# vmskisme/f_renderer

Hardware: AMD Instinct MI355X
Metric: Mtri/s (and Mfrag/s), 1M-triangle frame @1920x1080 (higher is better)
Workload: dtype f32; 1 GPU; random_1M_tris_1920x1080_depth; scene=1M random clip-space triangles, 1920x1080, depth-only, width=1920, height=1080, triangles=1000000, setup_triangles=1000052, covered_fragments=60715175, varyings=0, tile=32x32, frames_in_flight=2, partition=tile rows in 1 contiguous block(s)

## Files before the change

f_renderer_amd/csrc/frr_raster.h:

```cpp
#pragma once
#include "frr_device.h"
#ifndef __HIPCC_RTC__
#include <type_traits>
#endif

namespace frr {

__device__ __forceinline__ int xcd_remap(int bid, int nwg)
{
    const int q = nwg / 8, r = nwg % 8, xcd = bid % 8;
    return (xcd < r ? xcd * (q + 1) : r * (q + 1) + (xcd - r) * q) + bid / 8;
}

__device__ __forceinline__ uint32_t order_id(const RasterArgs &a, uint32_t slot)
{
    const uint32_t nt = a.ntris_draw;
    return 1u + (slot < nt ? slot << FAN_BITS : a.fan_okey[slot - nt]);
}
__device__ __forceinline__ uint32_t id_slot(const RasterArgs &a, uint32_t id)
{
    const uint32_t okl = id - 1u, t = okl >> FAN_BITS, f = okl & ((1u << FAN_BITS) - 1u);
    return f ? a.ntris_draw + a.fanbase[t] + (f - 1u) : t;
}
__device__ __forceinline__ uint32_t id_emission(const RasterArgs &a, uint32_t tri_base, uint32_t id)
// ... 209 lines not shown
    const uint32_t A12 = 0u - (uint32_t)(p2y - p1y), B12 = (uint32_t)(p2x - p1x);
    const uint32_t A20 = 0u - (uint32_t)(p0y - p2y), B20 = (uint32_t)(p0x - p2x);
    const uint32_t E01o = A01 * (uint32_t)(bx0 - p0x) + B01 * (uint32_t)(by0 - p0y);
    const uint32_t E12o = A12 * (uint32_t)(bx0 - p1x) + B12 * (uint32_t)(by0 - p1y);
    const uint32_t E20o = A20 * (uint32_t)(bx0 - p2x) + B20 * (uint32_t)(by0 - p2y);
    const uint32_t fl = r->flags;
    const int thr01 = (fl & 2u) ? 0 : -1, thr12 = (fl & 4u) ? 0 : -1, thr20 = (fl & 8u) ? 0 : -1;
    const float r0 = r->rhw[0], r1 = r->rhw[1], r2 = r->rhw[2];
    const float inv_bw = __builtin_amdgcn_rcpf((float)bw);
    const unsigned long long idlow = (unsigned long long)key_id;
    for (int p = lane; p < npx; p += 64) {
        const int dy = (int)(((float)p + 0.5f) * inv_bw);
        const int dx = p - __mul24(dy, bw);
        const int E01 = (int)(E01o + A01 * (uint32_t)dx + B01 * (uint32_t)dy);
        const int E12 = (int)(E12o + A12 * (uint32_t)dx + B12 * (uint32_t)dy);
        const int E20 = (int)(E20o + A20 * (uint32_t)dx + B20 * (uint32_t)dy);
        bool covered = (E01 > thr01) & (E12 > thr12) & (E20 > thr20);
        const int cx = bx0 + dx, cy = by0 + dy;
        const int pix = (cy - c.ay0) * TILE + (cx - c.ax0);
        if (NANPASS) {
            const uint32_t last_nan = nanL[pix];
            covered = covered && last_nan != 0u && key_id > last_nan;
        } else {
            n_cov += (uint32_t)__popcll(__ballot(covered));
        }
        if (covered) {
            Frag f = frag_eval(s0x, s0y, s1x, s1y, s2x, s2y, r0, r1, r2, cx, cy);
            if (f.valid) {
                const bool isnan = f.rhw != f.rhw;
                if (NANPASS) {
                    if (!isnan) atomicMax(&s_key[pix], ((unsigned long long)zkey(f.rhw) << 32) | idlow);
                } else {
                    if (isnan) { ++n_nan; *nanflag = 1u; }
                    atomicMax(&s_key[pix], ((unsigned long long)zkey_frag(f.rhw) << 32) | idlow);
                }
            }
        }
    }
}

__device__ __forceinline__ void tile_nan_begin(const TileCtx &c, unsigned long long *s_key, uint32_t *nanL)
{
    for (int i = threadIdx.x; i < TILE_PX; i += (int)blockDim.x) {
        const int x = i & (TILE - 1), y = i >> 5;
        const unsigned long long k = s_key[i];
        const bool nanpix = x < c.tw && y < c.th && (uint32_t)(k >> 32) == ZKEY_NAN_FRAG;
        nanL[i] = nanpix ? (uint32_t)k : 0u;
        if (nanpix) s_key[i] = ((unsigned long long)ZKEY_NAN_BELOW << 32) | (unsigned long long)(uint32_t)k;
    }
}

template <int K, int PS>
__global__ __launch_bounds__(256) void k_raster(RasterArgs a, DevUniforms u)
{
    __shared__ unsigned long long s_key[TILE_PX];
    __shared__ uint32_t s_nanL[TILE_PX];
    __shared__ uint32_t s_nanflag;
    if (seq_cancelled(a.cnt, a.seq, a.epoch, true)) return;
    const TileCtx c = tile_ctx(a);
    if (c.beg >= c.end) return;
    tile_load_keys(a, c, s_key);
    if (threadIdx.x == 0) s_nanflag = 0u;
    __syncthreads();
    const int lane = threadIdx.x & 63;
    const uint32_t wave = __builtin_amdgcn_readfirstlane(threadIdx.x >> 6);
    uint32_t n_cov = 0, n_nan = 0;
    for (uint32_t e = c.beg + wave; e < c.end; e += 4) {
        const uint32_t t = __builtin_amdgcn_readfirstlane(a.bins[e].x);
        sweep_triangle(a, c, t, order_id(a, t), lane, s_key, n_cov, n_nan, &s_nanflag);
    }
    if (lane == 0 && n_cov) atomicAdd(&a.cnt->lane[a.lane].gtab[a.gpar].frag_covered, (unsigned long long)n_cov);
    if (n_nan) atomicAdd(&a.cnt->lane[a.lane].gtab[a.gpar].frag_nan, (unsigned long long)n_nan);
    __syncthreads();
    if (s_nanflag != 0u) {
        tile_nan_begin(c, s_key, s_nanL);
        __syncthreads();
        for (uint32_t e = c.beg + wave; e < c.end; e += 4) {
            const uint32_t t = __builtin_amdgcn_readfirstlane(a.bins[e].x);
            sweep_triangle<true>(a, c, t, order_id(a, t), lane, s_key, n_cov, n_nan, nullptr, s_nanL);
        }
        __syncthreads();
    }
    tile_resolve<K, PS>(a, u, c, s_key);
}

template <int K, int PS>
__global__ __launch_bounds__(256) void k_raster_entries(RasterArgs a, DevUniforms u)
{
    if (seq_cancelled(a.cnt, a.seq, a.epoch, true)) return;
    const GeomTab *g = gtab_of(a);
    const uint32_t n = g->n_emit, tri_base = g->tri_base;
    const long long nent = (long long)(a.win_h - 1) * a.dstride + a.win_w;
    const long long e = (long long)blockIdx.x * 256 + threadIdx.x;
    if (e >= nent) return;
    const int ex = (int)(e % a.dstride), ey = (int)(e / a.dstride);
    const int kmax = (a.win_w - 1 - ex) / a.dstride;
    float depth = a.depth[e];
    uint32_t id = 0u, n_cov = 0u, n_nan = 0u;
    bool wrote = false;
    for (uint32_t i = 0; i < n; ++i) {
        const uint32_t t = slot_of_emission(a, i);
        const RasterRec *__restrict__ r = a.recs + t;
        const float s0x = r->s[0], s0y = r->s[1], s1x = r->s[2], s1y = r->s[3], s2x = r->s[4], s2y = r->s[5];
        const int p0x = f32_as_i32(s0x + 0.5f), p0y = f32_as_i32(s0y + 0.5f), p1x = f32_as_i32(s1x + 0.5f), p1y = f32_as_i32(s1y + 0.5f);
        const int p2x = f32_as_i32(s2x + 0.5f), p2y = f32_as_i32(s2y + 0.5f);
        const int bx0 = clampi(min(p0x, min(p1x, p2x)), a.x0, a.x1), bx1 = clampi(max(p0x, max(p1x, p2x)), a.x0, a.x1);
        const int by0 = clampi(min(p0y, min(p1y, p2y)), a.y0, a.y1), by1 = clampi(max(p0y, max(p1y, p2y)), a.y0, a.y1);
        if (bx1 <= bx0 || by1 <= by0) continue;
        const uint32_t A01 = 0u - (uint32_t)(p1y - p0y), B01 = (uint32_t)(p1x - p0x);
        const uint32_t A12 = 0u - (uint32_t)(p2y - p1y), B12 = (uint32_t)(p2x - p1x);
        const uint32_t A20 = 0u - (uint32_t)(p0y - p2y), B20 = (uint32_t)(p0x - p2x);
        const uint32_t fl = r->flags;
        const int thr01 = (fl & 2u) ? 0 : -1, thr12 = (fl & 4u) ? 0 : -1, thr20 = (fl & 8u) ? 0 : -1;
        const float r0 = r->rhw[0], r1 = r->rhw[1], r2 = r->rhw[2];
        for (int k = kmax; k >= 0; --k) {
            const int lx = ex + k * a.dstride, ly = ey - k;
            if (ly < 0 || ly >= a.win_h) continue;
            const int cx = a.x0 + lx, cy = a.y0 + ly;
            if (cx < bx0 || cx >= bx1 || cy < by0 || cy >= by1) continue;
            const int E01 = (int)(A01 * (uint32_t)(cx - p0x) + B01 * (uint32_t)(cy - p0y));
            const int E12 = (int)(A12 * (uint32_t)(cx - p1x) + B12 * (uint32_t)(cy - p1y));
            const int E20 = (int)(A20 * (uint32_t)(cx - p2x) + B20 * (uint32_t)(cy - p2y));
            if (!((E01 > thr01) & (E12 > thr12) & (E20 > thr20))) continue;
            ++n_cov;
            const Frag f = frag_eval(s0x, s0y, s1x, s1y, s2x, s2y, r0, r1, r2, cx, cy);
            if (!f.valid) continue;
            if (f.rhw != f.rhw) ++n_nan;
            if (f.rhw < depth) continue;
            depth = f.rhw; id = tri_base + i; wrote = true;
            if constexpr (PS != FRR_PS_DEPTH) {
                const float w = recip_exact(f.rhw != 0.0f ? f.rhw : 1.0f);
                const float c0 = r0 * f.a * w, c1 = r1 * f.b * w, c2 = r2 * f.c * w;
                float in[K > 0 ? K : 1];
                if constexpr (K > 0) {
                    const float *v = a.vary + (size_t)t * (3 * K);
#pragma unroll
                    for (int q = 0; q < K; ++q) in[q] = v[q] * c0 + v[K + q] * c1 + v[2 * K + q] * c2;
                }
                float col[4];
                run_ps<PS>(u, in, col, nullptr);
                reinterpret_cast<uint32_t *>(a.color)[(size_t)ly * a.cstride + lx] =
                    quantize_u8(col[0]) | (quantize_u8(col[1]) << 8) | (quantize_u8(col[2]) << 16) | (quantize_u8(col[3]) << 24);
            }
        }
    }
    if (wrote) { a.depth[e] = depth; a.tri_id[e] = id; }
    if (n_cov) atomicAdd(&a.cnt->lane[a.lane].gtab[a.gpar].frag_covered, (unsigned long long)n_cov);
    if (n_nan) atomicAdd(&a.cnt->lane[a.lane].gtab[a.gpar].frag_nan, (unsigned long long)n_nan);
}

constexpr int SPAN_SAFE = 8191;
constexpr int SPAN_BATCH = 32;
#ifndef FRR_SPAN_CULL
#define FRR_SPAN_CULL 32
#endif
constexpr int SPAN_CULL = FRR_SPAN_CULL;
#ifndef FRR_SPAN_AQ_MIN
#define FRR_SPAN_AQ_MIN 1
#endif
#ifndef FRR_LIGHT_NW
#define FRR_LIGHT_NW 3
#endif
#ifndef FRR_LIGHT_B
#define FRR_LIGHT_B 32
#endif
constexpr int LIGHT_NW = FRR_LIGHT_NW;
constexpr int LIGHT_B = FRR_LIGHT_B;
constexpr int SPAN_AQ_MIN = FRR_SPAN_AQ_MIN;

__device__ __forceinline__ void wave_lds_fence()
{
    __builtin_amdgcn_fence(__ATOMIC_ACQ_REL, "wavefront");
}

__device__ __forceinline__ int seg_rank(uint32_t h_lo, uint32_t h_hi, uint32_t le_lo, uint32_t le_hi, int base)
{
    return __popc(h_hi & le_hi) + (__popc(h_lo & le_lo) + base);
}
struct alignas(16) SpanTri {
    int32_t m01, m12, m20;
    uint32_t zub;
    uint32_t kd01, kd12, kd20;
    uint32_t misc;
    float r01, r12, r20, pad;
};
__device__ __forceinline__ void span_edge_bound(int m, uint32_t kd, float rD, int pmask, int row, int &lo, int &hi)
{
    const int k = (int)(kd << 16) >> 16, D = (int)(kd >> 16);
    const int M = m + __mul24(k, row);
    int q = (int)__builtin_amdgcn_fmed3f((float)M * rD, -2.0f, 40.0f);
    const int r = M - __mul24(q, D);
    q += (r >> 31) + (int)(r >= D);
    lo = max(lo, q & pmask);
    hi = min(hi, max(q + 1, pmask & 64));
}

constexpr int DIRECT_MAX = 256;
#ifndef FRR_DIRECT_STEPS
#define FRR_DIRECT_STEPS 2
#endif
constexpr int DIRECT_STEPS = FRR_DIRECT_STEPS;
constexpr int DIRECT_MIN = 4;
constexpr int HZ_SEG = 0, HZ_BLK = 128, HZ_QUAD = 144, HZ_C4 = 148, HZ_SIZE = 404;
#ifndef FRR_BKT_LOG2
#define FRR_BKT_LOG2 6
#endif
constexpr int BKT_LOG2 = FRR_BKT_LOG2, BKT_N = 1 << BKT_LOG2, BKT_SHIFT = 27 - BKT_LOG2, BKT_PER = BKT_N / 64;
__device__ __forceinline__ uint32_t z_bucket(uint32_t zub_key) { return (uint32_t)(BKT_N - 1) - ((zub_key >> BKT_SHIFT) & (uint32_t)(BKT_N - 1)); }
__device__ __forceinline__ void bucket_scan(uint32_t *s_bkt, int lane, uint32_t base)
{
    uint32_t v[BKT_PER], sum = 0u;
#pragma unroll
    for (int j = 0; j < BKT_PER; ++j) { v[j] = s_bkt[lane * BKT_PER + j]; sum += v[j]; }
    uint32_t run = base + wave_incl_scan_dpp(sum) - sum;
#pragma unroll
    for (int j = 0; j < BKT_PER; ++j) { s_bkt[lane * BKT_PER + j] = run; run += v[j]; }
}
__device__ __forceinline__ uint32_t dpp_xor1(uint32_t v) { return (uint32_t)__builtin_amdgcn_update_dpp(0, (int)v, 0xB1, 0xf, 0xf, false); }
__device__ __forceinline__ uint32_t dpp_xor2(uint32_t v) { return (uint32_t)__builtin_amdgcn_update_dpp(0, (int)v, 0x4E, 0xf, 0xf, false); }

__device__ __forceinline__ void hiz_rebuild(const unsigned long long *s_key, uint32_t *hz, int lane)
{
    const uint4 *p = reinterpret_cast<const uint4 *>(s_key);
    uint32_t m[8];
#pragma unroll
    for (int k = 0; k < 8; ++k) { const uint4 v = p[64 * k + lane]; m[k] = min(v.y, v.w); }
    uint32_t c4[8], sg[8];
#pragma unroll
    for (int k = 0; k < 8; ++k) {
        c4[k] = min(m[k], dpp_xor1(m[k]));
        sg[k] = min(c4[k], dpp_xor2(c4[k]));
    }
#pragma unroll
    for (int k = 0; k < 8; ++k) {
        if ((lane & 1) == 0) hz[HZ_C4 + 32 * k + (lane >> 1)] = c4[k] >> 1;
        if ((lane & 3) == 0) hz[HZ_SEG + 16 * k + (lane >> 2)] = sg[k];
    }
    __builtin_amdgcn_fence(__ATOMIC_ACQ_REL, "wavefront");
    if (lane < 16) {
        const int by = lane >> 2, bx = lane & 3;
        uint32_t mm = 0xFFFFFFFFu;
#pragma unroll
        for (int r = 0; r < 8; ++r) mm = min(mm, hz[HZ_SEG + (by * 8 + r) * 4 + bx]);
        hz[HZ_BLK + lane] = mm;
    }
    __builtin_amdgcn_fence(__ATOMIC_ACQ_REL, "wavefront");
    if (lane < 4) {
        const int qy = lane >> 1, qx = lane & 1;
        const uint32_t *b = hz + HZ_BLK + (qy * 2) * 4 + qx * 2;
        hz[HZ_QUAD + lane] = min(min(b[0], b[1]), min(b[4], b[5]));
    }
}

template <int NW, int B> struct SpanLds {
    static constexpr int KEY = 0;
    static constexpr int U0 = KEY + TILE_PX * 8;
    static constexpr int TRI = U0;
    static constexpr int FA = TRI + NW * B * 48;
    static constexpr int FB = FA + NW * B * 16;
    static constexpr int FC = FB + NW * B * 16;
    static constexpr int HROW = FC + NW * B * 8;
    static constexpr int HFRAG = HROW + NW * (B / 2) * 8;
    static constexpr int Q = HFRAG + NW * 32 * 8;
    static constexpr int M_END = Q + NW * 64 * 4;
    static constexpr int SEGPRE = U0;
    static constexpr int SEGSRC = SEGPRE + ((BIN_MAX_G + 1 + 3) & ~3) * 4;
    static constexpr int EXCH = SEGSRC + BIN_MAX_G * 4;
    static constexpr int P_END = EXCH + DIRECT_MAX * 16;
    static constexpr int U1 = M_END > P_END ? M_END : P_END;
    static constexpr int HZ = U1;
    static constexpr int BKT = HZ + ((HZ_SIZE + 3) & ~3) * 4;
    static constexpr int SCAL = BKT + BKT_N * 4;
    static constexpr int U8 = SCAL + 8 * 4;
    static constexpr int bytes(bool textured) { return U8 + (textured ? 256 * 4 : 0); }
};

template <int K, int PS, bool COUNT, int NW, int OCC>
__global__ __launch_bounds__(NW * 64, OCC) void k_raster_span(RasterArgs a, DevUniforms u, int win_safe)
{
    constexpr int B = NW <= 3 ? LIGHT_B : (OCC >= 8 || NW >= 16) ? 16 : SPAN_BATCH;
    constexpr bool TEXTURED = PS == FRR_PS_PHONG || PS == FRR_PS_BLINN || PS >= FRR_SHADER_USER_BASE;
    static_assert(B <= 32, "staging slots are five bits of a span descriptor, first rows ten bits of SpanTri::misc");
    using L = SpanLds<NW, B>;
    __shared__ __attribute__((aligned(16))) unsigned char s_raw[L::bytes(TEXTURED)];
    unsigned long long *const s_key = reinterpret_cast<unsigned long long *>(s_raw + L::KEY);
    SpanTri (*const s_tri)[B] = reinterpret_cast<SpanTri (*)[B]>(s_raw + L::TRI);
    float4 (*const s_fa)[B] = reinterpret_cast<float4 (*)[B]>(s_raw + L::FA);
    float4 (*const s_fb)[B] = reinterpret_cast<float4 (*)[B]>(s_raw + L::FB);
    float2 (*const s_fc)[B] = reinterpret_cast<float2 (*)[B]>(s_raw + L::FC);
    unsigned long long (*const s_hrow)[B / 2] = reinterpret_cast<unsigned long long (*)[B / 2]>(s_raw + L::HROW);
    unsigned long long (*const s_hfrag)[32] = reinterpret_cast<unsigned long long (*)[32]>(s_raw + L::HFRAG);
    uint32_t (*const s_q)[64] = reinterpret_cast<uint32_t (*)[64]>(s_raw + L::Q);
    uint32_t *const s_segpre = reinterpret_cast<uint32_t *>(s_raw + L::SEGPRE);
    uint32_t *const s_segsrc = reinterpret_cast<uint32_t *>(s_raw + L::SEGSRC);
    uint4 *const s_exch = reinterpret_cast<uint4 *>(s_raw + L::EXCH);
    uint32_t *const s_hz = reinterpret_cast<uint32_t *>(s_raw + L::HZ);
    uint32_t *const s_bkt = reinterpret_cast<uint32_t *>(s_raw + L::BKT);
    uint32_t &s_next = *reinterpret_cast<uint32_t *>(s_raw + L::SCAL);
    uint32_t &s_dirty = *reinterpret_cast<uint32_t *>(s_raw + L::SCAL + 4);
    uint32_t &s_ebase = *reinterpret_cast<uint32_t *>(s_raw + L::SCAL + 8);
    uint32_t &s_nanflag = *reinterpret_cast<uint32_t *>(s_raw + L::SCAL + 12);
    uint32_t *const s_nanL = reinterpret_cast<uint32_t *>(s_raw + L::U0);
    static_assert(L::U1 - L::U0 >= TILE_PX * 4, "the NaN pass keeps one u32 per pixel in the staging region");
    uint32_t *const s_w4 = reinterpret_cast<uint32_t *>(s_raw + L::SCAL + 16);
    float *const s_u8 = reinterpret_cast<float *>(s_raw + L::U8);
    if (TEXTURED) for (int i = threadIdx.x; i < 256; i += NW * 64) s_u8[i] = (float)i / 255.0f;
    const int lane = threadIdx.x & 63;
    const int w = __builtin_amdgcn_readfirstlane(threadIdx.x >> 6);
#ifdef FRR_DEBUG_COUNTERS
    unsigned long long d_tlast = __builtin_amdgcn_s_memtime();
    const unsigned long long d_rt0 = __builtin_amdgcn_s_memrealtime();
    unsigned long long d_rt1 = 0, d_rt2 = 0;
    uint32_t d_t[8] = {0, 0, 0, 0, 0, 0, 0, 0};
#define FRR_T(i) do { const unsigned long long now_ = __builtin_amdgcn_s_memtime(); d_t[i] += (uint32_t)(now_ - d_tlast); d_tlast = now_; } while (0)
#else
#define FRR_T(i) do { } while (0)
#endif
    __builtin_amdgcn_s_setprio(3);
    const uint32_t first_bad = seq_first_bad(a.cnt);
    TileCtx c = tile_ctx(a);
    const bool segmented = a.nseg != 0;
    if (!segmented && seq_is_cancelled(first_bad, a.seq, a.epoch, true)) return;
    if (segmented) {
        uint32_t s0 = 0, cn = 0;
        if (threadIdx.x < a.nseg) {
            const uint32_t *r = a.seg + (size_t)threadIdx.x * ((size_t)gridDim.x + 1) + c.ltile;
            s0 = r[0];
            cn = r[1] - s0;
        }
        if (seq_is_cancelled(first_bad, a.seq, a.epoch, true)) return;
        const uint32_t inc = wave_incl_scan_dpp(cn);
        if (lane == 63 && w < 4) s_w4[w] = inc;
        uint32_t s0x = 0, cnx = 0, incx = 0;
        if (NW == 3 && w == 0) {
            if (192u + (uint32_t)lane < a.nseg) {
                const uint32_t *r = a.seg + (size_t)(192 + lane) * ((size_t)gridDim.x + 1) + c.ltile;
                s0x = r[0];
                cnx = r[1] - s0x;
            }
            incx = wave_incl_scan_dpp(cnx);
            if (lane == 63) s_w4[3] = incx;
        }
        if (NW < 3 && threadIdx.x == 0) { s_w4[2] = 0u; s_w4[3] = 0u; }
        __syncthreads();
        const uint32_t w0 = s_w4[0], w1 = s_w4[1], w2 = s_w4[2], w3 = s_w4[3];
        const uint32_t total = __builtin_amdgcn_readfirstlane((w0 + w1) + (w2 + w3));
        if (threadIdx.x == 0 && a.tile_cost) a.tile_cost[c.ltile] = total;
        if (total == 0u) { tile_fill_clear(a, c); return; }
        if (threadIdx.x < BIN_MAX_G) {
            s_segpre[threadIdx.x] = (w > 0 ? w0 : 0u) + (w > 1 ? w1 : 0u) + (w > 2 ? w2 : 0u) + inc - cn;
            s_segsrc[threadIdx.x] = s0;
        }
        if (NW == 3 && w == 0) { s_segpre[192 + lane] = (w0 + w1) + w2 + incx - cnx; s_segsrc[192 + lane] = s0x; }
        if (NW < 3) for (int i = threadIdx.x + NW * 64; i < BIN_MAX_G; i += NW * 64) { s_segpre[i] = total; s_segsrc[i] = 0u; }
        if (threadIdx.x == 0) {
            s_segpre[BIN_MAX_G] = total;
            const uint32_t ntiles = gridDim.x;
            s_ebase = total <= a.ent_slot ? (uint32_t)c.ltile * a.ent_slot
                                          : ntiles * a.ent_slot + atomicAdd(&a.cnt->lane[a.lane].btab[a.bpar].ent_cursor, total);
        }
        __syncthreads();
        c.beg = __builtin_amdgcn_readfirstlane(s_ebase);
        c.end = c.beg + total;
    } else if (c.beg >= c.end) {
        tile_fill_clear(a, c);
        return;
    }
    auto source = [&](uint32_t k) -> uint4 {
        if (!segmented) return a.bins[c.beg + k];
        uint32_t g = 0;
#pragma unroll
        for (int st = BIN_MAX_G / 2; st >= 1; st >>= 1) if (s_segpre[g + st] <= k) g += st;
        return a.bins[s_segsrc[g] + (k - s_segpre[g])];
    };
    tile_load_keys(a, c, s_key, ~0ull);
    const uint32_t hz0 = a.fused_clear ? zkey_depth(a.clear_depth) : 0u;
    if (threadIdx.x == 0) { s_next = 0; s_dirty = a.fused_clear ? 0u : 1u; s_nanflag = 0u; }
    for (int i = threadIdx.x; i < BKT_N; i += NW * 64) s_bkt[i] = 0;
    for (int i = threadIdx.x; i < HZ_SIZE; i += NW * 64) s_hz[i] = i >= HZ_C4 ? hz0 >> 1 : hz0;
    __syncthreads();

    uint4 *__restrict__ ents = a.bins2;
    const uint32_t nent = c.end - c.beg;
    const bool direct = nent <= (uint32_t)(DIRECT_MAX < NW * 64 ? DIRECT_MAX : NW * 64);
    uint4 dent = make_uint4(0, 0, 0, 0);
    bool dvalid = false;
    int dcount = 0, dpos = 0, dstep = 64;
    if (direct) {
        const bool have = threadIdx.x < nent;
        const uint4 rec = have ? source(threadIdx.x) : make_uint4(0, 0, 0, 0);
        const uint32_t bkt = COUNT ? 0u : z_bucket(rec.y);
        if (have) atomicAdd(&s_bkt[bkt], 1u);
        __syncthreads();
        if (w == 0) bucket_scan(s_bkt, lane, 0u);
        __syncthreads();
        uint4 *const exch = s_exch;
        if (have) exch[atomicAdd(&s_bkt[bkt], 1u)] = rec;
        __syncthreads();
        const uint32_t q = (uint32_t)lane * NW + (uint32_t)w;
        dvalid = q < nent;
        if (dvalid) dent = exch[q];
        dcount = __popcll(__ballot(dvalid));
        dstep = max(DIRECT_MIN, (dcount + DIRECT_STEPS - 1) / DIRECT_STEPS);
        __syncthreads();
    } else {
        const bool sorted = !COUNT && nent > 2u * B;
        auto bucket_of = [&](const uint4 &e) { return sorted ? z_bucket(e.y) : 0u; };
        uint4 ce[4];
#pragma unroll
        for (int k = 0; k < 4; ++k) {
            const uint32_t e = threadIdx.x + (uint32_t)(NW * 64) * k;
            ce[k] = make_uint4(0, 0, 0, 0);
            if (e < nent) { ce[k] = source(e); atomicAdd(&s_bkt[bucket_of(ce[k])], 1u); }
        }
        for (uint32_t e = threadIdx.x + 4u * NW * 64; e < nent; e += NW * 64) atomicAdd(&s_bkt[bucket_of(source(e))], 1u);
        __syncthreads();
        if (w == 0) bucket_scan(s_bkt, lane, c.beg);
        __syncthreads();
#pragma unroll
        for (int k = 0; k < 4; ++k) {
            const uint32_t e = threadIdx.x + (uint32_t)(NW * 64) * k;
            if (e < nent) ents[atomicAdd(&s_bkt[bucket_of(ce[k])], 1u)] = ce[k];
        }
        for (uint32_t e = threadIdx.x + 4u * NW * 64; e < nent; e += NW * 64) {
            const uint4 en = source(e);
            ents[atomicAdd(&s_bkt[bucket_of(en)], 1u)] = en;
        }
        __builtin_amdgcn_fence(__ATOMIC_RELEASE, "workgroup");
        __syncthreads();
        __builtin_amdgcn_fence(__ATOMIC_ACQUIRE, "workgroup");
    }

    __builtin_amdgcn_s_setprio(0);
    const uint32_t le_lo = lane < 32 ? (2u << lane) - 1u : 0xFFFFFFFFu;
    const uint32_t le_hi = lane < 32 ? 0u : (2u << (lane - 32)) - 1u;
    uint32_t n_cov = 0, n_nan = 0;
#ifdef FRR_DEBUG_COUNTERS
    uint32_t d_tri = 0, d_alive = 0, d_rows = 0, d_spans = 0, d_spans_live = 0, d_frags = 0, d_fwin = 0, d_rwin = 0;
    uint32_t d_pre = 0, d_win = 0, d_rebuild = 0;
#endif

    constexpr int CULL = SPAN_CULL < B ? SPAN_CULL : B;
    if (direct) {
        const int nsteps = max(DIRECT_STEPS, (dcount + B - 1) / B);
        dstep = max(min(DIRECT_MIN, B), (dcount + nsteps - 1) / nsteps);
    }
    FRR_T(0);
#ifdef FRR_DEBUG_COUNTERS
    d_rt1 = __builtin_amdgcn_s_memrealtime();
#endif
    for (;;) {
        uint32_t e0 = 0;
        int dlo = 0;
        if (direct) {
            dlo = dpos;
            dpos += dstep;
            if (dlo >= dcount) break;
        } else {
            uint32_t b = 0;
            if (lane == 0) b = atomicAdd(&s_next, 1u);
            b = __builtin_amdgcn_readfirstlane(b);
            e0 = c.beg + b * (uint32_t)CULL;
            if (e0 >= c.end) break;
        }
        if (__builtin_amdgcn_readfirstlane(s_dirty) != 0u) {
            FRR_T(1);
            if (lane == 0) s_dirty = 0u;
            hiz_rebuild(s_key, s_hz, lane);
#ifdef FRR_DEBUG_COUNTERS
            ++d_rebuild;
#endif
            FRR_T(2);
        }
        wave_lds_fence();
        const bool valid = direct ? (dvalid && lane >= dlo && lane < dlo + dstep) : lane < (int)min((uint32_t)CULL, c.end - e0);
        const uint4 en = direct ? dent : (valid ? ents[e0 + lane] : make_uint4(0, 0, 0, 0));
        const int mnx = (int)(short)(en.z & 0xFFFFu), mny = (int)(short)(en.z >> 16);
        const int mxx = (int)(short)(en.w & 0xFFFFu), mxy = (int)(short)(en.w >> 16);
        const int bx0 = max(clampi(mnx, a.x0, a.x1), c.ax0), bx1 = min(clampi(mxx, a.x0, a.x1), c.ax0 + c.tw);
        const int by0 = max(clampi(mny, a.y0, a.y1), c.ay0), by1 = min(clampi(mxy, a.y0, a.y1), c.ay0 + c.th);
        const bool nonempty = valid && bx1 > bx0 && by1 > by0;
        const int amax = max(max(abs(mnx), abs(mxx)), max(abs(mny), abs(mxy)));
        const bool safe = nonempty && win_safe && amax <= SPAN_SAFE;
        bool alive = safe;
        if (!COUNT && safe) {
            const int gx0 = (bx0 - c.ax0) >> 3, gx1 = (bx1 - 1 - c.ax0) >> 3, gy0 = (by0 - c.ay0) >> 3, gy1 = (by1 - 1 - c.ay0) >> 3;
            const bool small = gx1 - gx0 <= 1 && gy1 - gy0 <= 1;
            const uint32_t *lv = s_hz + (small ? HZ_BLK : HZ_QUAD);
            const int sh = small ? 0 : 1, st = small ? 4 : 2;
            const int ix0 = gx0 >> sh, ix1 = gx1 >> sh, iy0 = gy0 >> sh, iy1 = gy1 >> sh;
            const uint32_t hm = min(min(lv[iy0 * st + ix0], lv[iy0 * st + ix1]), min(lv[iy1 * st + ix0], lv[iy1 * st + ix1]));
            alive = !(en.y < hm);
        }
#ifdef FRR_DEBUG_COUNTERS
        d_tri += __popcll(__ballot(nonempty)); d_alive += __popcll(__ballot(alive));
#endif
        unsigned long long um = __ballot(nonempty && !safe);
        while (um) {
            const int src = __builtin_ctzll(um);
            um &= um - 1;
            const uint32_t tu = (uint32_t)__builtin_amdgcn_readlane((int)en.x, src);
            uint32_t ncv = 0;
            sweep_triangle(a, c, tu, PS == FRR_PS_DEPTH ? emission_id(a, tu) : order_id(a, tu), lane, s_key, ncv, n_nan, &s_nanflag);
            n_cov += ncv;
        }
        const unsigned long long am = __ballot(alive);
        FRR_T(1);
        if (am == 0ull) continue;
        const int trank = (int)__builtin_amdgcn_mbcnt_hi((uint32_t)(am >> 32), __builtin_amdgcn_mbcnt_lo((uint32_t)am, 0u));
        const uint32_t rows = alive ? (uint32_t)(by1 - by0) : 0u;
        const uint32_t rincl = wave_incl_scan_dpp(rows);
        if (alive) {
            const uint4 *rp = reinterpret_cast<const uint4 *>(a.recs + en.x);
            const uint4 q0 = rp[0], q1 = rp[1], q2 = rp[2], q3 = rp[3];
            auto m_of = [&](uint32_t kd, uint32_t cc) { return (int)cc + __mul24((int)(kd << 16) >> 16, by0) - __mul24((int)(kd >> 16), bx0); };
            auto r_of = [&](uint32_t kd) { return fminf(__builtin_amdgcn_rcpf((float)(kd >> 16)), 64.0f); };
            SpanTri t;
            t.m01 = m_of(q0.x, q0.y); t.m12 = m_of(q0.z, q0.w); t.m20 = m_of(q1.x, q1.y);
            t.zub = en.y;
            t.kd01 = q0.x; t.kd12 = q0.z; t.kd20 = q1.x;
            t.misc = (uint32_t)(bx0 - c.ax0) | ((uint32_t)(by0 - c.ay0) << 5) | ((uint32_t)(bx1 - bx0) << 10) |
                     (((q3.w >> REC_POS_SHIFT) & 7u) << 16) | ((rincl - rows) << 19);
            t.r01 = r_of(q0.x); t.r12 = r_of(q0.z); t.r20 = r_of(q1.x);
            t.pad = 0.0f;
            s_tri[w][trank] = t;
            s_fa[w][trank] = make_float4(u2f(q1.z), u2f(q1.w), u2f(q2.x), u2f(q2.y));
            s_fb[w][trank] = make_float4(u2f(q2.z), u2f(q2.w), u2f(q3.x), u2f(q3.y));
            s_fc[w][trank] = make_float2(u2f(q3.z), u2f(PS == FRR_PS_DEPTH ? emission_id_rec(a, en.x, q3.w) : order_id(a, en.x)));
        }
        const int R = (int)__builtin_amdgcn_readlane((int)rincl, 63);
        if (lane < B / 2) s_hrow[w][lane] = 0ull;
        wave_lds_fence();
        if (rows) {
            const uint32_t st = rincl - rows;
            atomicOr(reinterpret_cast<uint32_t *>(&s_hrow[w][0]) + (st >> 5), 1u << (st & 31));
        }
        wave_lds_fence();
        const unsigned long long hrow_mine = s_hrow[w][lane & (B / 2 - 1)];
        wave_lds_fence();

        int jbase = 0;
        FRR_T(3);
        for (int r0 = 0; r0 < R; r0 += 64) {
            const uint32_t h_lo = (uint32_t)__builtin_amdgcn_readlane((int)(uint32_t)hrow_mine, r0 >> 6);
            const uint32_t h_hi = (uint32_t)__builtin_amdgcn_readlane((int)(uint32_t)(hrow_mine >> 32), r0 >> 6);
            const bool ractive = r0 + lane < R;
            const int j = seg_rank(h_lo, h_hi, le_lo, le_hi, jbase - 1);
            int len = 0, xl = 0, yl = 0;
            uint32_t zu = 0xFFFFFFFFu;
            if (ractive) {
                const SpanTri ti = s_tri[w][j];
                const int row = r0 + lane - (int)(ti.misc >> 19);
                const int bwj = (int)((ti.misc >> 10) & 63u);
                int lo = 0, hi = bwj;
                span_edge_bound(ti.m01, ti.kd01, ti.r01, (int)(ti.misc << 15) >> 31, row, lo, hi);
                span_edge_bound(ti.m12, ti.kd12, ti.r12, (int)(ti.misc << 14) >> 31, row, lo, hi);
                span_edge_bound(ti.m20, ti.kd20, ti.r20, (int)(ti.misc << 13) >> 31, row, lo, hi);
                len = max(hi - lo, 0);
                xl = (int)(ti.misc & 31u) + lo;
                yl = (int)((ti.misc >> 5) & 31u) + row;
                zu = ti.zub;
            }
#ifdef FRR_DEBUG_COUNTERS
            d_rwin++; d_rows += __popcll(__ballot(ractive)); d_spans += __popcll(__ballot(len > 0));
#endif
            jbase += __popc(h_lo) + __popc(h_hi);
            if (COUNT) n_cov += (uint32_t)__builtin_amdgcn_readlane((int)wave_incl_scan_dpp((uint32_t)len), 63);
            if (len > 0) {
                const uint4 ca = *reinterpret_cast<const uint4 *>(&s_hz[HZ_C4 + yl * 8]);
                const uint4 cb = *reinterpret_cast<const uint4 *>(&s_hz[HZ_C4 + yl * 8 + 4]);
                const uint32_t zh = zu >> 1;
                uint32_t cm = 0u;
                cm = __builtin_amdgcn_alignbit(cm, zh - cb.w, 31); cm = __builtin_amdgcn_alignbit(cm, zh - cb.z, 31);
                cm = __builtin_amdgcn_alignbit(cm, zh - cb.y, 31); cm = __builtin_amdgcn_alignbit(cm, zh - cb.x, 31);
                cm = __builtin_amdgcn_alignbit(cm, zh - ca.w, 31); cm = __builtin_amdgcn_alignbit(cm, zh - ca.z, 31);
                cm = __builtin_amdgcn_alignbit(cm, zh - ca.y, 31); cm = __builtin_amdgcn_alignbit(cm, zh - ca.x, 31);
                const int xr = xl + len - 1;
                const int c0 = xl >> 2, c1 = xr >> 2;
                const uint32_t pm = ~cm & ((2u << c1) - (1u << c0));
                if (pm == 0u) {
                    len = 0;
                } else {
                    const int f = __builtin_ctz(pm), l = 31 - __builtin_clz(pm);
                    const int nxl = max(xl, f << 2), nxr = min(xr, (l << 2) + 3);
                    xl = nxl;
                    len = nxr - nxl + 1;
                }
            }
            const unsigned long long nz = __ballot(len > 0);
#ifdef FRR_DEBUG_COUNTERS
            d_spans_live += __popcll(nz);
#endif
            if (nz == 0ull) { FRR_T(4); continue; }
            const int srank = (int)__builtin_amdgcn_mbcnt_hi((uint32_t)(nz >> 32), __builtin_amdgcn_mbcnt_lo((uint32_t)nz, 0u));
            const uint32_t fincl = wave_incl_scan_dpp((uint32_t)len);
            const int F = (int)__builtin_amdgcn_readlane((int)fincl, 63);
            if (lane < 32) s_hfrag[w][lane] = 0ull;
            wave_lds_fence();
            if (len > 0) {
                const uint32_t st = fincl - (uint32_t)len;
                atomicOr(reinterpret_cast<uint32_t *>(&s_hfrag[w][0]) + (st >> 5), 1u << (st & 31));
                s_q[w][srank] = (uint32_t)j | ((uint32_t)yl << 5) | (((uint32_t)xl + 2048u - st) << 10);
            }
            wave_lds_fence();
            const unsigned long long hfrag_mine = s_hfrag[w][lane & 31];

#ifdef FRR_DEBUG_COUNTERS
            d_frags += F; d_fwin += (F + 63) / 64;
#endif
            int qbase = 0;
            FRR_T(4);
            for (int f0 = 0; f0 < F; f0 += 64) {
                const uint32_t g_lo = (uint32_t)__builtin_amdgcn_readlane((int)(uint32_t)hfrag_mine, f0 >> 6);
                const uint32_t g_hi = (uint32_t)__builtin_amdgcn_readlane((int)(uint32_t)(hfrag_mine >> 32), f0 >> 6);
                if (f0 + lane < F) {
                    const uint32_t d = s_q[w][seg_rank(g_lo, g_hi, le_lo, le_hi, qbase - 1)];
                    const int sj = (int)(d & 31u), y = (int)((d >> 5) & 31u), x = (int)(d >> 10) + (f0 - 2048) + lane;
                    const float4 fa = s_fa[w][sj], fb = s_fb[w][sj];
                    const float2 fc = s_fc[w][sj];
                    Frag f = frag_eval(fa.x, fa.y, fa.z, fa.w, fb.x, fb.y, fb.z, fb.w, fc.x, c.ax0 + x, c.ay0 + y);
                    if (f.valid) {
                        if (f.rhw != f.rhw) { ++n_nan; s_nanflag = 1u; }
                        const unsigned long long key = ((unsigned long long)zkey_frag(f.rhw) << 32) | (unsigned long long)f2u(fc.y);
#ifdef FRR_DEBUG_COUNTERS
                        const unsigned long long old = atomicMax(&s_key[y * TILE + x], key);
                        d_pre += __popcll(__ballot(s_tri[w][sj].zub < (uint32_t)(old >> 32)));
                        d_win += __popcll(__ballot(key > old));
#else
                        atomicMax(&s_key[y * TILE + x], key);
#endif
                    }
                }
                qbase += __popc(g_lo) + __popc(g_hi);
            }
            if (lane == 0) s_dirty = 1u;
            wave_lds_fence();
            FRR_T(5);
        }

        wave_lds_fence();
    }
    FRR_T(1);
    if (lane == 0 && n_cov) atomicAdd(&a.cnt->lane[a.lane].gtab[a.gpar].frag_covered, (unsigned long long)n_cov);
#ifdef FRR_DEBUG_COUNTERS
    d_rt2 = __builtin_amdgcn_s_memrealtime();
    if (lane == 0) {
        unsigned long long *d = a.cnt->dbg[blockIdx.x % DBG_COPIES];
        atomicAdd(d + 0, (unsigned long long)d_tri); atomicAdd(d + 1, (unsigned long long)d_alive); atomicAdd(d + 2, (unsigned long long)d_rows);
        atomicAdd(d + 3, (unsigned long long)d_spans); atomicAdd(d + 4, (unsigned long long)d_spans_live); atomicAdd(d + 5, (unsigned long long)d_frags);
        atomicAdd(d + 6, (unsigned long long)d_fwin); atomicAdd(d + 7, (unsigned long long)d_rwin);
        atomicAdd(d + 8, (unsigned long long)d_pre); atomicAdd(d + 9, (unsigned long long)d_win); atomicAdd(d + 10, (unsigned long long)d_rebuild);
    }
#endif
    if (n_nan) atomicAdd(&a.cnt->lane[a.lane].gtab[a.gpar].frag_nan, (unsigned long long)n_nan);
    __syncthreads();
    if (s_nanflag != 0u) {
        tile_nan_begin(c, s_key, s_nanL);
        __syncthreads();
        uint32_t dummy_cov = 0, dummy_nan = 0;
        if (direct) {
            unsigned long long m = __ballot(dvalid);
            while (m) {
                const int src = __builtin_ctzll(m);
                m &= m - 1;
                const uint32_t tu = (uint32_t)__builtin_amdgcn_readlane((int)dent.x, src);
                sweep_triangle<true>(a, c, tu, PS == FRR_PS_DEPTH ? emission_id(a, tu) : order_id(a, tu), lane, s_key, dummy_cov, dummy_nan, nullptr, s_nanL);
            }
        } else {
            for (uint32_t e = c.beg + (uint32_t)w; e < c.end; e += NW) {
                const uint32_t tu = __builtin_amdgcn_readfirstlane(ents[e].x);
                sweep_triangle<true>(a, c, tu, PS == FRR_PS_DEPTH ? emission_id(a, tu) : order_id(a, tu), lane, s_key, dummy_cov, dummy_nan, nullptr, s_nanL);
            }
        }
        __syncthreads();
    }
    FRR_T(6);
    if constexpr (PS == FRR_PS_DEPTH) tile_resolve_depth4(a, c, s_key);
    else tile_resolve<K, PS>(a, u, c, s_key, TEXTURED ? s_u8 : nullptr);
#ifdef FRR_DEBUG_COUNTERS
    FRR_T(7);
    if (lane == 0) {
        unsigned long long *d = a.cnt->dbg[blockIdx.x % DBG_COPIES];
#pragma unroll
        for (int i = 0; i < 8; ++i) atomicAdd(d + 12 + i, (unsigned long long)d_t[i]);
        atomicAdd(d + 20, 1ull);
        if (a.dbg_tiles && w == 0) {
            unsigned long long *tl = a.dbg_tiles + (size_t)c.ltile * 8;
            tl[0] = d_rt0; tl[1] = d_rt1; tl[2] = d_rt2; tl[3] = __builtin_amdgcn_s_memrealtime();
            tl[4] = (unsigned long long)__builtin_amdgcn_s_getreg(4 | (31 << 11)) | ((unsigned long long)__builtin_amdgcn_s_getreg(20 | (31 << 11)) << 32);
            tl[5] = (unsigned long long)(c.end - c.beg) | ((unsigned long long)(uint32_t)c.tile << 32);
            tl[6] = d_t[1] + d_t[3] + d_t[4] + d_t[5]; tl[7] = d_t[0] | ((unsigned long long)blockIdx.x << 32);
        }
    }
#endif
#undef FRR_T
}

__global__ void k_debug_scan(const uint32_t *in, uint32_t *out)
{
    out[threadIdx.x] = wave_incl_scan_dpp(in[threadIdx.x]);
}

}
```

Before: 11150 Mtri/s.

## Terminate tile batch loop early using per-bucket suffix max depth vs tile HiZ minimum

While bucketing entries by depth, the change also records each bucket's maximum depth key, with a flag bit for triangles outside the safe range. It then builds a suffix maximum per group of buckets and keeps the tile-wide HiZ minimum up to date in hiz_rebuild. Before processing a batch, if every remaining entry is provably occluded by the current tile depth, it moves the batch counter to the end and skips the rest. This removes culling work on the occluded tail of front-to-back sorted tiles, at the cost of extra LDS atomics and scratch space.

```diff
diff --git a/f_renderer_amd/csrc/frr_raster.h b/f_renderer_amd/csrc/frr_raster.h
--- a/f_renderer_amd/csrc/frr_raster.h
+++ b/f_renderer_amd/csrc/frr_raster.h
@@ -440,19 +440,31 @@
 #endif
 constexpr int BKT_LOG2 = FRR_BKT_LOG2, BKT_N = 1 << BKT_LOG2, BKT_SHIFT = 27 - BKT_LOG2, BKT_PER = BKT_N / 64;
 __device__ __forceinline__ uint32_t z_bucket(uint32_t zub_key) { return (uint32_t)(BKT_N - 1) - ((zub_key >> BKT_SHIFT) & (uint32_t)(BKT_N - 1)); }
-__device__ __forceinline__ void bucket_scan(uint32_t *s_bkt, int lane, uint32_t base)
+__device__ __forceinline__ void bucket_scan(const uint32_t *s_bkt, uint32_t *out, int lane, uint32_t base)
 {
     uint32_t v[BKT_PER], sum = 0u;
 #pragma unroll
     for (int j = 0; j < BKT_PER; ++j) { v[j] = s_bkt[lane * BKT_PER + j]; sum += v[j]; }
     uint32_t run = base + wave_incl_scan_dpp(sum) - sum;
 #pragma unroll
-    for (int j = 0; j < BKT_PER; ++j) { s_bkt[lane * BKT_PER + j] = run; run += v[j]; }
+    for (int j = 0; j < BKT_PER; ++j) { out[lane * BKT_PER + j] = run; run += v[j]; }
+}
+__device__ __forceinline__ void bucket_suffix_max(const uint32_t *s_zmax, uint32_t *out, int lane, bool valid)
+{
+    uint32_t v = 0u;
+#pragma unroll
+    for (int j = 0; j < BKT_PER; ++j) v = max(v, s_zmax[lane * BKT_PER + j]);
+#pragma unroll
+    for (int d = 1; d < 64; d <<= 1) {
+        const uint32_t o = (uint32_t)__shfl_down((int)v, d);
+        v = max(v, o);
+    }
+    out[lane] = valid ? v : 0xFFFFFFFFu;
 }
 __device__ __forceinline__ uint32_t dpp_xor1(uint32_t v) { return (uint32_t)__builtin_amdgcn_update_dpp(0, (int)v, 0xB1, 0xf, 0xf, false); }
 __device__ __forceinline__ uint32_t dpp_xor2(uint32_t v) { return (uint32_t)__builtin_amdgcn_update_dpp(0, (int)v, 0x4E, 0xf, 0xf, false); }
 
-__device__ __forceinline__ void hiz_rebuild(const unsigned long long *s_key, uint32_t *hz, int lane)
+__device__ __forceinline__ void hiz_rebuild(const unsigned long long *s_key, uint32_t *hz, uint32_t *tmin, int lane)
 {
     const uint4 *p = reinterpret_cast<const uint4 *>(s_key);
     uint32_t m[8];
@@ -481,7 +493,11 @@
     if (lane < 4) {
         const int qy = lane >> 1, qx = lane & 1;
         const uint32_t *b = hz + HZ_BLK + (qy * 2) * 4 + qx * 2;
-        hz[HZ_QUAD + lane] = min(min(b[0], b[1]), min(b[4], b[5]));
+        const uint32_t q = min(min(b[0], b[1]), min(b[4], b[5]));
+        hz[HZ_QUAD + lane] = q;
+        const uint32_t q2 = min(q, dpp_xor1(q));
+        const uint32_t q4 = min(q2, dpp_xor2(q2));
+        if (lane == 0) *tmin = q4;
     }
 }
 
@@ -499,7 +515,9 @@
     static constexpr int SEGPRE = U0;
     static constexpr int SEGSRC = SEGPRE + ((BIN_MAX_G + 1 + 3) & ~3) * 4;
     static constexpr int EXCH = SEGSRC + BIN_MAX_G * 4;
-    static constexpr int P_END = EXCH + DIRECT_MAX * 16;
+    static constexpr int CUR = EXCH + DIRECT_MAX * 16;
+    static constexpr int ZMAX = CUR + BKT_N * 4;
+    static constexpr int P_END = ZMAX + BKT_N * 4;
     static constexpr int U1 = M_END > P_END ? M_END : P_END;
     static constexpr int HZ = U1;
     static constexpr int BKT = HZ + ((HZ_SIZE + 3) & ~3) * 4;
@@ -536,6 +554,9 @@
     uint32_t *const s_nanL = reinterpret_cast<uint32_t *>(s_raw + L::U0);
     static_assert(L::U1 - L::U0 >= TILE_PX * 4, "the NaN pass keeps one u32 per pixel in the staging region");
     uint32_t *const s_w4 = reinterpret_cast<uint32_t *>(s_raw + L::SCAL + 16);
+    uint32_t *const s_cur = reinterpret_cast<uint32_t *>(s_raw + L::CUR);
+    uint32_t *const s_zmax = reinterpret_cast<uint32_t *>(s_raw + L::ZMAX);
+    uint32_t &s_tmin = s_w4[0];
     float *const s_u8 = reinterpret_cast<float *>(s_raw + L::U8);
     if (TEXTURED) for (int i = threadIdx.x; i < 256; i += NW * 64) s_u8[i] = (float)i / 255.0f;
     const int lane = threadIdx.x & 63;
@@ -608,8 +629,8 @@
     };
     tile_load_keys(a, c, s_key, ~0ull);
     const uint32_t hz0 = a.fused_clear ? zkey_depth(a.clear_depth) : 0u;
-    if (threadIdx.x == 0) { s_next = 0; s_dirty = a.fused_clear ? 0u : 1u; s_nanflag = 0u; }
-    for (int i = threadIdx.x; i < BKT_N; i += NW * 64) s_bkt[i] = 0;
+    if (threadIdx.x == 0) { s_next = 0; s_dirty = a.fused_clear ? 0u : 1u; s_nanflag = 0u; s_tmin = hz0; }
+    for (int i = threadIdx.x; i < BKT_N; i += NW * 64) { s_bkt[i] = 0; s_zmax[i] = 0; }
     for (int i = threadIdx.x; i < HZ_SIZE; i += NW * 64) s_hz[i] = i >= HZ_C4 ? hz0 >> 1 : hz0;
     __syncthreads();
 
@@ -625,7 +646,7 @@
         const uint32_t bkt = COUNT ? 0u : z_bucket(rec.y);
         if (have) atomicAdd(&s_bkt[bkt], 1u);
         __syncthreads();
-        if (w == 0) bucket_scan(s_bkt, lane, 0u);
+        if (w == 0) bucket_scan(s_bkt, s_bkt, lane, 0u);
         __syncthreads();
         uint4 *const exch = s_exch;
         if (have) exch[atomicAdd(&s_bkt[bkt], 1u)] = rec;
@@ -639,25 +660,36 @@
     } else {
         const bool sorted = !COUNT && nent > 2u * B;
         auto bucket_of = [&](const uint4 &e) { return sorted ? z_bucket(e.y) : 0u; };
+        auto count = [&](const uint4 &e) {
+            const uint32_t bkt = bucket_of(e);
+            atomicAdd(&s_bkt[bkt], 1u);
+            if (sorted) {
+                const int lo = min((int)(short)(e.z & 0xFFFFu), (int)(short)(e.z >> 16)), hi = max((int)(short)(e.w & 0xFFFFu), (int)(short)(e.w >> 16));
+                atomicMax(&s_zmax[bkt], e.y | (uint32_t)(min(lo + SPAN_SAFE, SPAN_SAFE - hi) >> 31));
+            }
+        };
         uint4 ce[4];
 #pragma unroll
         for (int k = 0; k < 4; ++k) {
             const uint32_t e = threadIdx.x + (uint32_t)(NW * 64) * k;
             ce[k] = make_uint4(0, 0, 0, 0);
-            if (e < nent) { ce[k] = source(e); atomicAdd(&s_bkt[bucket_of(ce[k])], 1u); }
-        }
-        for (uint32_t e = threadIdx.x + 4u * NW * 64; e < nent; e += NW * 64) atomicAdd(&s_bkt[bucket_of(source(e))], 1u);
-        __syncthreads();
-        if (w == 0) bucket_scan(s_bkt, lane, c.beg);
+            if (e < nent) { ce[k] = source(e); count(ce[k]); }
+        }
+        for (uint32_t e = threadIdx.x + 4u * NW * 64; e < nent; e += NW * 64) count(source(e));
+        __syncthreads();
+        if (w == 0) {
+            bucket_scan(s_bkt, s_cur, lane, c.beg);
+            if (!COUNT) bucket_suffix_max(s_zmax, s_bkt, lane, sorted && win_safe);
+        }
         __syncthreads();
 #pragma unroll
         for (int k = 0; k < 4; ++k) {
             const uint32_t e = threadIdx.x + (uint32_t)(NW * 64) * k;
-            if (e < nent) ents[atomicAdd(&s_bkt[bucket_of(ce[k])], 1u)] = ce[k];
+            if (e < nent) ents[atomicAdd(&s_cur[bucket_of(ce[k])], 1u)] = ce[k];
         }
         for (uint32_t e = threadIdx.x + 4u * NW * 64; e < nent; e += NW * 64) {
             const uint4 en = source(e);
-            ents[atomicAdd(&s_bkt[bucket_of(en)], 1u)] = en;
+            ents[atomicAdd(&s_cur[bucket_of(en)], 1u)] = en;
         }
         __builtin_amdgcn_fence(__ATOMIC_RELEASE, "workgroup");
         __syncthreads();
@@ -699,7 +731,7 @@
         if (__builtin_amdgcn_readfirstlane(s_dirty) != 0u) {
             FRR_T(1);
             if (lane == 0) s_dirty = 0u;
-            hiz_rebuild(s_key, s_hz, lane);
+            hiz_rebuild(s_key, s_hz, &s_tmin, lane);
 #ifdef FRR_DEBUG_COUNTERS
             ++d_rebuild;
 #endif
@@ -708,6 +740,15 @@
         wave_lds_fence();
         const bool valid = direct ? (dvalid && lane >= dlo && lane < dlo + dstep) : lane < (int)min((uint32_t)CULL, c.end - e0);
         const uint4 en = direct ? dent : (valid ? ents[e0 + lane] : make_uint4(0, 0, 0, 0));
+        if (!COUNT && !direct) {
+            const uint32_t fb = z_bucket(__builtin_amdgcn_readfirstlane(en.y)) / (uint32_t)BKT_PER;
+            if (__ballot(s_bkt[fb] < s_tmin) != 0ull) {
+                uint32_t left = c.end - e0;
+                asm volatile("" : "+s"(left));
+                __hip_atomic_store(&s_next, (e0 - c.beg) / (uint32_t)CULL + (left + (uint32_t)CULL - 1u) / (uint32_t)CULL, __ATOMIC_RELAXED, __HIP_MEMORY_SCOPE_WORKGROUP);
+                continue;
+            }
+        }
         const int mnx = (int)(short)(en.z & 0xFFFFu), mny = (int)(short)(en.z >> 16);
         const int mxx = (int)(short)(en.w & 0xFFFFu), mxy = (int)(short)(en.w >> 16);
         const int bx0 = max(clampi(mnx, a.x0, a.x1), c.ax0), bx1 = min(clampi(mxx, a.x0, a.x1), c.ax0 + c.tw);
```

Result: slower. 10650 Mtri/s (-4.5%).

## Cull 64-entry batches per wave and drain survivors in B-sized sub-steps

Applied to the files above, without the earlier changes.

Raises the span-cull step from 32 to 64 entries, so one wave Hi-Z tests a full 64-lane batch at once. Survivors are then processed in chunks of B, and the leftover mask is carried into further loop iterations. Between chunks, the Hi-Z is rebuilt when it is dirty and the remaining entries are re-tested, so more triangles get culled. This amortises the atomic fetch and cull per step, at the cost of added loop control, extra ballots and possibly more Hi-Z rebuilds. It also adds a readfirstlane on the direct-mode step counter, an asm barrier in hiz_rebuild, and extra debug counters.

```diff
diff --git a/f_renderer_amd/csrc/frr_raster.h b/f_renderer_amd/csrc/frr_raster.h
--- a/f_renderer_amd/csrc/frr_raster.h
+++ b/f_renderer_amd/csrc/frr_raster.h
@@ -385,9 +385,14 @@
 constexpr int SPAN_SAFE = 8191;
 constexpr int SPAN_BATCH = 32;
 #ifndef FRR_SPAN_CULL
-#define FRR_SPAN_CULL 32
+#define FRR_SPAN_CULL 64
 #endif
 constexpr int SPAN_CULL = FRR_SPAN_CULL;
+static_assert(SPAN_CULL >= 1 && SPAN_CULL <= 64, "a step's records are the lanes of one wave");
+#ifndef FRR_SPAN_RETEST
+#define FRR_SPAN_RETEST 1
+#endif
+constexpr bool SPAN_RETEST = FRR_SPAN_RETEST != 0;
 #ifndef FRR_SPAN_AQ_MIN
 #define FRR_SPAN_AQ_MIN 1
 #endif
@@ -454,6 +459,7 @@
 
 __device__ __forceinline__ void hiz_rebuild(const unsigned long long *s_key, uint32_t *hz, int lane)
 {
+    asm volatile("" : "+v"(lane));
     const uint4 *p = reinterpret_cast<const uint4 *>(s_key);
     uint32_t m[8];
 #pragma unroll
@@ -671,9 +677,11 @@
 #ifdef FRR_DEBUG_COUNTERS
     uint32_t d_tri = 0, d_alive = 0, d_rows = 0, d_spans = 0, d_spans_live = 0, d_frags = 0, d_fwin = 0, d_rwin = 0;
     uint32_t d_pre = 0, d_win = 0, d_rebuild = 0;
-#endif
-
-    constexpr int CULL = SPAN_CULL < B ? SPAN_CULL : B;
+    uint32_t d_steps = 0, d_requl = 0;
+#endif
+
+    constexpr int CULL = (B == 32 && NW >= 4) ? SPAN_CULL : (SPAN_CULL < B ? SPAN_CULL : B);
+    constexpr bool BATCHED = CULL > B;
     if (direct) {
         const int nsteps = max(DIRECT_STEPS, (dcount + B - 1) / B);
         dstep = max(min(DIRECT_MIN, B), (dcount + nsteps - 1) / nsteps);
@@ -687,7 +695,7 @@
         int dlo = 0;
         if (direct) {
             dlo = dpos;
-            dpos += dstep;
+            dpos = __builtin_amdgcn_readfirstlane(dpos + dstep);
             if (dlo >= dcount) break;
         } else {
             uint32_t b = 0;
@@ -696,18 +704,31 @@
             e0 = c.beg + b * (uint32_t)CULL;
             if (e0 >= c.end) break;
         }
-        if (__builtin_amdgcn_readfirstlane(s_dirty) != 0u) {
+#ifdef FRR_DEBUG_COUNTERS
+        ++d_steps;
+#endif
+        unsigned long long rem = 0ull;
+        if (BATCHED) rem = __ballot(direct ? (dvalid && lane >= dlo && lane < dlo + dstep) : lane < (int)min((uint32_t)CULL, c.end - e0));
+        bool test = true;
+#ifdef FRR_DEBUG_COUNTERS
+        bool d_first = true;
+#endif
+        do {
+        if ((SPAN_RETEST || test) && __builtin_amdgcn_readfirstlane(s_dirty) != 0u) {
             FRR_T(1);
             if (lane == 0) s_dirty = 0u;
             hiz_rebuild(s_key, s_hz, lane);
+            test = true;
 #ifdef FRR_DEBUG_COUNTERS
             ++d_rebuild;
 #endif
             FRR_T(2);
         }
         wave_lds_fence();
-        const bool valid = direct ? (dvalid && lane >= dlo && lane < dlo + dstep) : lane < (int)min((uint32_t)CULL, c.end - e0);
-        const uint4 en = direct ? dent : (valid ? ents[e0 + lane] : make_uint4(0, 0, 0, 0));
+        bool valid;
+        if (BATCHED) valid = (((lane < 32 ? (uint32_t)rem : (uint32_t)(rem >> 32)) >> (lane & 31)) & 1u) != 0u;
+        else valid = direct ? (dvalid && lane >= dlo && lane < dlo + dstep) : lane < (int)min((uint32_t)CULL, c.end - e0);
+        const uint4 en = direct ? dent : (valid ? (ents + e0)[(uint32_t)lane] : make_uint4(0, 0, 0, 0));
         const int mnx = (int)(short)(en.z & 0xFFFFu), mny = (int)(short)(en.z >> 16);
         const int mxx = (int)(short)(en.w & 0xFFFFu), mxy = (int)(short)(en.w >> 16);
         const int bx0 = max(clampi(mnx, a.x0, a.x1), c.ax0), bx1 = min(clampi(mxx, a.x0, a.x1), c.ax0 + c.tw);
@@ -716,7 +737,7 @@
         const int amax = max(max(abs(mnx), abs(mxx)), max(abs(mny), abs(mxy)));
         const bool safe = nonempty && win_safe && amax <= SPAN_SAFE;
         bool alive = safe;
-        if (!COUNT && safe) {
+        if (!COUNT && safe && (!BATCHED || test)) {
             const int gx0 = (bx0 - c.ax0) >> 3, gx1 = (bx1 - 1 - c.ax0) >> 3, gy0 = (by0 - c.ay0) >> 3, gy1 = (by1 - 1 - c.ay0) >> 3;
             const bool small = gx1 - gx0 <= 1 && gy1 - gy0 <= 1;
             const uint32_t *lv = s_hz + (small ? HZ_BLK : HZ_QUAD);
@@ -726,7 +747,9 @@
             alive = !(en.y < hm);
         }
 #ifdef FRR_DEBUG_COUNTERS
-        d_tri += __popcll(__ballot(nonempty)); d_alive += __popcll(__ballot(alive));
+        if (d_first) { d_tri += __popcll(__ballot(nonempty)); d_alive += __popcll(__ballot(alive)); }
+        else d_requl += __popcll(__ballot(safe && !alive));
+        d_first = false;
 #endif
         unsigned long long um = __ballot(nonempty && !safe);
         while (um) {
@@ -737,10 +760,17 @@
             sweep_triangle(a, c, tu, PS == FRR_PS_DEPTH ? emission_id(a, tu) : order_id(a, tu), lane, s_key, ncv, n_nan, &s_nanflag);
             n_cov += ncv;
         }
-        const unsigned long long am = __ballot(alive);
+        unsigned long long am = __ballot(alive);
         FRR_T(1);
-        if (am == 0ull) continue;
+        if (am == 0ull) { rem = 0ull; continue; }
         const int trank = (int)__builtin_amdgcn_mbcnt_hi((uint32_t)(am >> 32), __builtin_amdgcn_mbcnt_lo((uint32_t)am, 0u));
+        if (BATCHED) {
+            alive = alive && trank < B;
+            const unsigned long long bm = __ballot(alive);
+            rem = am ^ bm;
+            am = bm;
+            test = false;
+        }
         const uint32_t rows = alive ? (uint32_t)(by1 - by0) : 0u;
         const uint32_t rincl = wave_incl_scan_dpp(rows);
         if (alive) {
@@ -872,6 +902,7 @@
         }
 
         wave_lds_fence();
+        } while (BATCHED && rem != 0ull);
     }
     FRR_T(1);
     if (lane == 0 && n_cov) atomicAdd(&a.cnt->lane[a.lane].gtab[a.gpar].frag_covered, (unsigned long long)n_cov);
@@ -883,6 +914,7 @@
         atomicAdd(d + 3, (unsigned long long)d_spans); atomicAdd(d + 4, (unsigned long long)d_spans_live); atomicAdd(d + 5, (unsigned long long)d_frags);
         atomicAdd(d + 6, (unsigned long long)d_fwin); atomicAdd(d + 7, (unsigned long long)d_rwin);
         atomicAdd(d + 8, (unsigned long long)d_pre); atomicAdd(d + 9, (unsigned long long)d_win); atomicAdd(d + 10, (unsigned long long)d_rebuild);
+        atomicAdd(d + 11, (unsigned long long)d_steps | ((unsigned long long)d_requl << 32));
     }
 #endif
     if (n_nan) atomicAdd(&a.cnt->lane[a.lane].gtab[a.gpar].frag_nan, (unsigned long long)n_nan);
```

Result: slower. 11400 Mtri/s before, 11090 Mtri/s after (-2.7%).
